# nianticlabs/panoptic-forecasting

Measured on AMD Instinct MI355X. Metric: forecast frames/sec @1024x2048, 3-in->dt=3 bg, higher is better.
Workload: dtype f32 as 2 fp16 terms/operand, 3 MFMA products, f32 accumulate (strict f32: fp32_only); 1 GPU; configs[1] bg short-term forecast 3-in dt=3 @1024x2048: 3 warp/splats + HarDNet-70 + upsample/argmax; resident_frames_per_gpu=128, streams=4, sub_batch=32, launch=hipGraph replay, sub-batches staggered, weights=random-init, calibrated (tests/golden/calib_seed1234.json), world=1, device=AMD Radeon Graphics, backend=single process

## Files before the change

include/pfhip.h:

```cpp
#ifndef PFHIP_H
#define PFHIP_H

#include <stddef.h>
#include <stdint.h>

#ifdef __cplusplus
extern "C" {
#endif

#define PF_OK 0
#define PF_EINVAL (-1)
#define PF_EWORKSPACE (-2)
#define PF_EBLOB (-3)
#define PF_EHIP (-4)
#define PF_EUNSUPPORTED (-5)

typedef struct pf_plan pf_plan;

int pf_version(void);
const char *pf_last_error(void);

#define PF_SPLAT_PER_FRAME 1
#define PF_SPLAT_PER_SAMPLE_SENTINEL 2
int pf_warp_splat_workspace(int B, int T, int H, int W, int per_frame, size_t *bytes);
// ... 128 lines not shown
int pf_train_param_count(const pf_train *t, size_t *n_floats);
int pf_train_param_layout(const pf_train *t, int op_index, size_t *w_off, size_t *aux_off, int *has_bn);
int pf_train_workspace(const pf_train *t, int B, int H, int W, int out_h, int out_w, size_t *bytes);
int pf_train_forward_backward(const pf_train *t, float *theta, float *grad, int accumulate_grads, const void *seg, int seg_is_i64,
                              const float *depth, const uint8_t *depth_mask, float depth_mean, float depth_std, int T,
                              const float *x_dense, int B, int H, int W, const void *labels, int labels_i64, int out_h, int out_w,
                              int ignore_index, float loss_scale, float bn_momentum, float bn_eps, int update_running_stats,
                              double *out3, void *ws, size_t ws_bytes, void *stream);
int pf_train_tensor_view(const pf_train *t, const char *name, int want_grad, int B, int H, int W, int out_h, int out_w,
                         size_t *ws_offset, int *channels, int *h, int *w);
int pf_sgd_workspace(size_t *bytes);
int pf_sgd_step(float *theta, float *grad, float *momentum_buf, const uint8_t *trainable, size_t n, float lr, float momentum,
                float weight_decay, float clip_norm, float clip_value, int first_step, void *ws, size_t ws_bytes, void *stream);

int pf_hardnet_tensor_view(const pf_plan *plan, const char *name, int B, int H, int W,
                           size_t *ws_offset, int *channels, int *h, int *w);
int pf_hardnet_tensor_read(const pf_plan *plan, const char *name, int B, int H, int W, const void *ws, float *dst, void *stream);
int pf_s4_pack(const float *src, void *dst, int B, int C, int H, int W, unsigned *status, void *stream);
int pf_s4_unpack(const void *src, float *dst, int B, int C, int H, int W, void *stream);
int pf_hardnet_flops(const pf_plan *plan, int H, int W, double *flops);

int pf_profile_enable(int on);
int pf_profile_collect(void);
int pf_profile_get(int i, char *label, size_t label_cap, int *launches, double *total_ms, double *flops,
                   double *bytes);

int pf_debug_force_conv(int kind, int p0, int p1, int p2);
int pf_debug_conv_decision(int ks, int stride, int cin, int cout, int hout, int wout, int B, int need, int flags, int rounds,
                           int *out, int cap);
int pf_debug_net_choice(int what, const int *iargs, int n_iargs, const float *fargs, int n_fargs, char *label, size_t label_cap,
                        long long *out, int cap);
int pf_debug_conv_ranges(int form, int ks, int kc, int pad, int n_src, int n_cases, const int *choff, const int *ch, const int *ctotal,
                         int src_begin, int src_end, int *out, size_t cap);
int pf_debug_pack_conv(int layout, int ks, int stride, int cin, int cout, int n_src, const int *choff, const int *ch, int pad_sources,
                       int rem, int tiles, int chunks, const float *w, float *out, size_t cap, size_t *n_floats);
int pf_debug_plan_arena(const void *blob, size_t bytes, int in_ch, int n_cls, float *out, size_t cap, size_t *n_floats,
                        long long *table, int table_ops);
int pf_debug_plan_tail(const void *blob, size_t bytes, int in_ch, int n_cls, float *out, size_t cap, size_t *n_floats,
                       long long *table, int table_ops);
int pf_debug_plan_down(const void *blob, size_t bytes, int in_ch, int n_cls, float *out, size_t cap, size_t *n_floats,
                       long long *table, int table_ops);
int pf_debug_plan_wide(int form, const void *blob, size_t bytes, int in_ch, int n_cls, float *out, size_t cap, size_t *n_floats,
                       long long *table, int table_ops);
int pf_debug_hardnet_schedule(const void *blob, size_t bytes, int in_ch, int n_cls, int B, int H, int W, int out_h, int out_w, int stem_T,
                              int table_batch, unsigned char *formats, int cap_formats, int *n_formats, long long *steps, int cap_steps,
                              int *n_steps);
int pf_debug_train_plan(const void *blob, size_t bytes, int in_ch, int n_cls, int B, int H, int W, int out_h, int out_w,
                        long long *regions, int cap_regions, int *n_regions, int *steps, int cap_steps, int *n_steps, int *slots_streams);
int pf_debug_fg_schedule(int N, int T_in, int T_out, int flags, long long *regions, int cap_regions, int *n_regions, long long *steps,
                         char *labels, int cap_steps, int *n_steps);
int pf_debug_label_scan_span(unsigned long long addr_a, unsigned long long addr_b, int esz_a, int esz_b, int align_a, int align_b,
                             unsigned long long n, int P, unsigned long long *out5);
int pf_debug_probe_read(long long *host64);

#ifdef __cplusplus
}
#endif
#endif
```

panoptic-forecasting_amd/csrc/warp_splat.hip:

```cpp
#include "pf_common.h"
#include "pf_prof.h"
#include <cstdlib>

#ifndef PF_PROBE
#define PF_PROBE 0
#endif
#if PF_PROBE
#define RPROBE(i) do { if (threadIdx.x == 0 && blockIdx.x == 100 && blockIdx.y == 1 && blockIdx.z == 0 && a.probe) a.probe[i] = wall_clock64(); } while (0)
#else
#define RPROBE(i) do { } while (0)
#endif

namespace pf {
long long *probe_buffer();

constexpr unsigned long long kEmpty = ~0ull;
constexpr int kThreads = 256;
constexpr int kRThreads = 512;
constexpr int kRMinWaves = 8;
constexpr int kRHalves = kRThreads / 256;
constexpr int kSrcTH = 16, kSrcTW = 64;
constexpr int kDstTH = 32, kDstTW = 128;
constexpr int kScan = 256;
constexpr int kScanBatches = 8;
constexpr int kListCap = 64;
constexpr int kFlight = 2;
constexpr int kIdFrameShift = 20;
constexpr int kZSlots = 64;

struct SplatArgs {
    const float *depth;
    const uint8_t *mask;
    const uint8_t *seg;
    const float *Kinv, *E, *Tt, *Einv, *K;
    int4 *bbox;
    unsigned *zmax_part;
    uint8_t *inv_mark;
    uint2 *proj;
    unsigned *count;
    unsigned *lists;
    uint8_t *out_seg;
    float *out_depth;
    long long *out_r2d;
    int B, T_total, t_first, T, H, W, C, per_frame;
    int zgroups_per_sample;
    int stx, sty;
    int dtx, dty;
    long long *probe;
};

__device__ __forceinline__ unsigned float_to_ordered(float f) {
    unsigned b = __float_as_uint(f);
    return (b & 0x80000000u) ? ~b : (b | 0x80000000u);
}
__device__ __forceinline__ float ordered_to_float(unsigned k) {
    return __uint_as_float((k & 0x80000000u) ? (k & 0x7FFFFFFFu) : ~k);
}

__device__ __forceinline__ float dot3(const float *m, float a, float b, float c) {
    float acc = 0.0f;
    acc = __fadd_rn(acc, __fmul_rn(m[0], a));
    acc = __fadd_rn(acc, __fmul_rn(m[1], b));
    acc = __fadd_rn(acc, __fmul_rn(m[2], c));
    return acc;
}
__device__ __forceinline__ float dot4(const float *m, float a, float b, float c, float d) {
    float acc = 0.0f;
    acc = __fadd_rn(acc, __fmul_rn(m[0], a));
    acc = __fadd_rn(acc, __fmul_rn(m[1], b));
    acc = __fadd_rn(acc, __fmul_rn(m[2], c));
    acc = __fadd_rn(acc, __fmul_rn(m[3], d));
    return acc;
}

// ... 135 lines not shown
        for (int k = 0; k < 4; ++k)
#pragma unroll
            for (int i = 0; i < 4; ++i) vv[k][i] = dot4(E + 4 * i, c[k][0], c[k][1], c[k][2], 1.0f);
    }
    {
        float Tm[16];
        fetch_rows(after(relaunder((const float *)pT), relaunder((const float *)pT), vv[3][3]), Tm);
#pragma unroll
        for (int k = 0; k < 4; ++k)
#pragma unroll
            for (int i = 0; i < 4; ++i) w[k][i] = dot4(Tm + 4 * i, vv[k][0], vv[k][1], vv[k][2], vv[k][3]);
    }
    {
        float Einv[16];
        fetch_rows(after(relaunder((const float *)pEinv), relaunder((const float *)pEinv), w[3][3]), Einv);
#pragma unroll
        for (int k = 0; k < 4; ++k)
#pragma unroll
            for (int i = 0; i < 4; ++i) e[k][i] = dot4(Einv + 4 * i, w[k][0], w[k][1], w[k][2], w[k][3]);
    }
    float K[9];
    fetch_rows(after(relaunder((const float *)pK), relaunder((const float *)pK), e[3][3]), K);
#pragma unroll
    for (int k = 0; k < 4; ++k) {
        const float px = __fdiv_rn(e[k][0], e[k][3]), py = __fdiv_rn(e[k][1], e[k][3]), z = __fdiv_rn(e[k][2], e[k][3]);
        const float q0 = dot3(K + 0, px, py, z), q1 = dot3(K + 3, px, py, z), q2 = dot3(K + 6, px, py, z);
        p[k] = finish(__fdiv_rn(q0, q2), __fdiv_rn(q1, q2), z, m[k], Wf, Hf);
    }
}

__device__ __forceinline__ void load4(const SplatArgs &a, long long base, int x, int y, float d[4], bool m[4]) {
    const long long i = base + (long long)y * a.W + x;
    if ((a.W & 3) == 0 && x + 3 < a.W) {
        const float4 dv = *reinterpret_cast<const float4 *>(a.depth + i);
        const uchar4 mv = *reinterpret_cast<const uchar4 *>(a.mask + i);
        d[0] = dv.x; d[1] = dv.y; d[2] = dv.z; d[3] = dv.w;
        m[0] = mv.x != 0; m[1] = mv.y != 0; m[2] = mv.z != 0; m[3] = mv.w != 0;
    } else {
#pragma unroll
        for (int k = 0; k < 4; ++k) {
            const bool in = x + k < a.W;
            d[k] = in ? a.depth[i + k] : 1.0f;
            m[k] = in ? a.mask[i + k] != 0 : false;
        }
    }
}

__global__ __launch_bounds__(kThreads) void bin_kernel(SplatArgs a) {
    const int tile = blockIdx.x, tl = blockIdx.y, b = blockIdx.z;
    const int t = a.t_first + tl;
    const int ty0 = (tile / a.stx) * kSrcTH, tx0 = (tile % a.stx) * kSrcTW;
    const long long N = (long long)a.H * a.W;
    const long long in_base = ((long long)b * a.T_total + t) * N;
    const int y = ty0 + (threadIdx.x >> 4), x = tx0 + (threadIdx.x & 15) * 4;
    float d[4] = {1.0f, 1.0f, 1.0f, 1.0f};
    bool m[4] = {false, false, false, false};
    if (y < a.H && x < a.W) load4(a, in_base, x, y, d, m);
    const GlobalF pKinv = (GlobalF)a.Kinv + b * 9, pK = (GlobalF)a.K + b * 9, pE = (GlobalF)a.E + b * 16, pEinv = (GlobalF)a.Einv + b * 16,
                  pT = (GlobalF)a.Tt + ((long long)b * a.T_total + t) * 16;
    const bool affine = camera_affine(pKinv, pE, pT, pEinv, pK);
    const bool skewfree = camera_skewfree(pKinv, pK);
    const int g = a.per_frame ? tl : 0, G = a.per_frame ? a.T : 1;
    uint8_t *mark = a.inv_mark + ((long long)b * G + g) * N;
    long long *r2d = a.out_r2d ? a.out_r2d + ((long long)b * a.T + tl) * N * 2 : nullptr;
    const float Wf = (float)a.W, Hf = (float)a.H;

    float zmax = -INFINITY;
    int bx0 = 0x7fffffff, by0 = 0x7fffffff, bx1 = -1, by1 = -1;
    if (y < a.H && x < a.W) {
        uint2 *pj = a.proj + ((long long)b * a.T + tl) * N + (long long)y * a.W + x;
        unsigned pk[8];
        Proj p4[4];
        const bool fast_done = affine && skewfree && project4_fast<true>(pKinv, pE, pT, pEinv, pK, x, y, d, m, Wf, Hf, p4);
        if (!fast_done) {
            project4_full(pKinv, pE, pT, pEinv, pK, x, y, d, m, Wf, Hf, p4);
        }
#pragma unroll
        for (int k = 0; k < 4; ++k) {
            if (x + k >= a.W) break;
            const Proj p = p4[k];
            zmax = fmaxf(zmax, p.z);
            pk[2 * k] = __float_as_uint(p.z);
            pk[2 * k + 1] = (unsigned)p.x0 | ((unsigned)p.y0 << 13) | ((unsigned)(p.x1 != p.x0) << 26) |
                            ((unsigned)(p.y1 != p.y0) << 27) | ((unsigned)p.valid << 28);
            if ((a.W & 3) != 0) pj[k] = make_uint2(pk[2 * k], pk[2 * k + 1]);
            if (r2d) {
                const long long n = (long long)y * a.W + x + k;
                r2d[n * 2] = p.x0;
                r2d[n * 2 + 1] = p.y0;
            }
            if (p.valid) {
                bx0 = min(bx0, p.x0); by0 = min(by0, p.y0);
                bx1 = max(bx1, p.x1); by1 = max(by1, p.y1);
            } else {
                const unsigned o00 = (unsigned)p.y0 * (unsigned)a.W + (unsigned)p.x0, dxo = (unsigned)(p.x1 - p.x0);
                const unsigned o10 = (unsigned)p.y1 * (unsigned)a.W + (unsigned)p.x0;
                if (dxo) {
                    __builtin_memcpy(mark + o00, "\1\1", 2);
                    if (o10 != o00) __builtin_memcpy(mark + o10, "\1\1", 2);
                } else {
                    mark[o00] = 1;
                    if (o10 != o00) mark[o10] = 1;
                }
            }
        }
        if ((a.W & 3) == 0) {
            reinterpret_cast<uint4 *>(pj)[0] = make_uint4(pk[0], pk[1], pk[2], pk[3]);
            reinterpret_cast<uint4 *>(pj)[1] = make_uint4(pk[4], pk[5], pk[6], pk[7]);
        }
    }
    typedef unsigned short u16x2 __attribute__((ext_vector_type(2)));
    typedef short i16x2 __attribute__((ext_vector_type(2)));
    u16x2 bmin = {(unsigned short)min(bx0, 0xFFFF), (unsigned short)min(by0, 0xFFFF)};
    i16x2 bmax = {(short)bx1, (short)by1};
#define PF_DPP_STEP(ctrl, rmask)                                                                                              \
    {                                                                                                                         \
        zmax = fmaxf(zmax, __int_as_float(__builtin_amdgcn_update_dpp(__float_as_int(zmax), __float_as_int(zmax), ctrl, rmask, 0xF, false))); \
        const int mn = __builtin_bit_cast(int, bmin), mx = __builtin_bit_cast(int, bmax);                                     \
        bmin = __builtin_elementwise_min(bmin, __builtin_bit_cast(u16x2, __builtin_amdgcn_update_dpp(mn, mn, ctrl, rmask, 0xF, false))); \
        bmax = __builtin_elementwise_max(bmax, __builtin_bit_cast(i16x2, __builtin_amdgcn_update_dpp(mx, mx, ctrl, rmask, 0xF, false))); \
    }
    PF_DPP_STEP(0xB1, 0xF)
    PF_DPP_STEP(0x4E, 0xF)
    PF_DPP_STEP(0x141, 0xF)
    PF_DPP_STEP(0x140, 0xF)
    PF_DPP_STEP(0x142, 0xA)
    PF_DPP_STEP(0x143, 0xC)
#undef PF_DPP_STEP
    __shared__ float zred[kThreads / 64];
    __shared__ int bred[kThreads / 64][2];
    if ((threadIdx.x & 63) == 63) {
        const int w = threadIdx.x >> 6;
        zred[w] = zmax;
        bred[w][0] = __builtin_bit_cast(int, bmin);
        bred[w][1] = __builtin_bit_cast(int, bmax);
    }
    __syncthreads();
    zmax = zred[0];
    bmin = __builtin_bit_cast(u16x2, bred[0][0]);
    bmax = __builtin_bit_cast(i16x2, bred[0][1]);
#pragma unroll
    for (int w = 1; w < kThreads / 64; ++w) {
        zmax = fmaxf(zmax, zred[w]);
        bmin = __builtin_elementwise_min(bmin, __builtin_bit_cast(u16x2, bred[w][0]));
        bmax = __builtin_elementwise_max(bmax, __builtin_bit_cast(i16x2, bred[w][1]));
    }
    bx0 = bmin[0] == 0xFFFF ? 0x7fffffff : (int)bmin[0];
    by0 = bmin[1] == 0xFFFF ? 0x7fffffff : (int)bmin[1];
    bx1 = bmax[0];
    by1 = bmax[1];
    if (threadIdx.x == 0) {
        const long long ntile = (long long)a.stx * a.sty;
        atomicMax(&a.zmax_part[(b * a.zgroups_per_sample + (a.per_frame ? tl : 0)) * kZSlots + ((tile + b) & (kZSlots - 1))], float_to_ordered(zmax));
        a.bbox[((long long)b * a.T + tl) * ntile + tile] = make_int4(bx0, by0, bx1, by1);
    }
    if (bx1 >= 0) {
        const int ndst = a.dtx * a.dty;
        const long long dbase = ((long long)b * G + g) * ndst;
        const unsigned id = ((unsigned)(a.per_frame ? 0 : tl) << kIdFrameShift) | (unsigned)tile;
        const int dtx0 = bx0 / kDstTW, dty0 = by0 / kDstTH;
        const int ntx = bx1 / kDstTW - dtx0 + 1, nt = ntx * (by1 / kDstTH - dty0 + 1);
        for (int j = threadIdx.x; j < nt; j += kThreads) {
            const long long dst = dbase + (dty0 + j / ntx) * a.dtx + dtx0 + j % ntx;
            const unsigned slot = atomicAdd(&a.count[dst], 1u);
            if (slot < (unsigned)kListCap) a.lists[dst * kListCap + slot] = id;
        }
    }
}

__global__ __launch_bounds__(kRThreads, kRMinWaves) void raster_kernel(SplatArgs a) {
    __shared__ unsigned long long zb[kDstTH * kDstTW];
    __shared__ unsigned short list[kScan * kScanBatches];
    __shared__ unsigned ent[kListCap];
    __shared__ int list_n;
    __shared__ float sentinel_s;

    const int dtile = blockIdx.x, g = blockIdx.y, b = blockIdx.z;
    const int G = a.per_frame ? a.T : 1, Tg = a.per_frame ? 1 : a.T;
    const int dy0 = (dtile / a.dtx) * kDstTH, dx0 = (dtile % a.dtx) * kDstTW;
    const int dy1 = min(dy0 + kDstTH, a.H) - 1, dx1 = min(dx0 + kDstTW, a.W) - 1;
    const long long N = (long long)a.H * a.W;
    const long long P = (long long)Tg * N;
    const int ntile = a.stx * a.sty;

    RPROBE(0);
    [[maybe_unused]] int n_hits_total = 0;
    for (int i = threadIdx.x; i < kDstTH * kDstTW; i += kRThreads) zb[i] = kEmpty;
    const int lt = threadIdx.x & 255, half = threadIdx.x >> 8;

    if (threadIdx.x < 64) {
        unsigned m = a.zmax_part[(b * a.zgroups_per_sample + (a.per_frame ? g : 0)) * kZSlots + threadIdx.x];
#pragma unroll
        for (int o = 32; o > 0; o >>= 1) m = max(m, (unsigned)__shfl_xor((int)m, o));
        if (threadIdx.x == 0) sentinel_s = __fadd_rn(ordered_to_float(m), 1.0f);
    }

    auto splat4 = [&](const unsigned (&pk)[8], int x, int y, unsigned ebase) {
        const unsigned e_first = ebase + (unsigned)y * (unsigned)a.W + (unsigned)x;
        const unsigned Pu1 = (unsigned)P;
#pragma unroll
        for (int k = 0; k < 4; ++k) {
            const unsigned f = pk[2 * k + 1];
            if (!((f >> 28) & 1u)) continue;
            const unsigned rx0 = (f & 8191u) - (unsigned)dx0, ry0 = ((f >> 13) & 8191u) - (unsigned)dy0;
            const unsigned fx = (f >> 26) & 1u, fy = (f >> 27) & 1u;
            const unsigned rx1 = rx0 + fx, ry1 = ry0 + fy;
            const bool in_x0 = rx0 < (unsigned)kDstTW, in_x1 = rx1 < (unsigned)kDstTW && fx != 0u;
            const bool in_y0 = ry0 < (unsigned)kDstTH, in_y1 = ry1 < (unsigned)kDstTH && fy != 0u;
            const unsigned e0 = e_first + (unsigned)k;
            const unsigned long long khi = (unsigned long long)pk[2 * k] << 32;
            if (in_x0 && in_y0) atomicMin(&zb[ry0 * kDstTW + rx0], khi | e0);
            if (in_x0 && in_y1) atomicMin(&zb[ry1 * kDstTW + rx0], khi | (e0 + Pu1));
            if (in_x1 && in_y0) atomicMin(&zb[ry0 * kDstTW + rx1], khi | (e0 + 2u * Pu1));
            if (in_x1 && in_y1) atomicMin(&zb[ry1 * kDstTW + rx1], khi | (e0 + 3u * Pu1));
        }
    };
    auto load4 = [&](const uint2 *pbase, int stx, int sty, unsigned (&pk)[8], int &x, int &y) {
        y = sty * kSrcTH + (lt >> 4);
        x = stx * kSrcTW + (lt & 15) * 4;
#pragma unroll
        for (int k = 0; k < 8; ++k) pk[k] = 0u;
        if (stx < 0 || y >= a.H || x >= a.W) return;
        const uint2 *pj = pbase + (long long)y * a.W + x;
        if ((a.W & 3) == 0) {
            const uint4 q0 = reinterpret_cast<const uint4 *>(pj)[0], q1 = reinterpret_cast<const uint4 *>(pj)[1];
            pk[0] = q0.x; pk[1] = q0.y; pk[2] = q0.z; pk[3] = q0.w;
            pk[4] = q1.x; pk[5] = q1.y; pk[6] = q1.z; pk[7] = q1.w;
        } else {
#pragma unroll
            for (int k = 0; k < 4; ++k) {
                const uint2 q = x + k < a.W ? pj[k] : make_uint2(0u, 0u);
                pk[2 * k] = q.x; pk[2 * k + 1] = q.y;
            }
        }
    };
    const int ndst = a.dtx * a.dty;
    const long long dslot = ((long long)b * G + g) * ndst + dtile;
    const unsigned cnt = a.count[dslot];
    if (cnt <= (unsigned)kListCap) {
        if (threadIdx.x < cnt) {
            const unsigned e = a.lists[dslot * kListCap + threadIdx.x], st = e & ((1u << kIdFrameShift) - 1u), row = st / (unsigned)a.stx;
            ent[threadIdx.x] = (e & ~((1u << kIdFrameShift) - 1u)) | (row << 10) | (st - row * (unsigned)a.stx);
        }
        __syncthreads();
        for (int li = 0; li < (int)cnt; li += kFlight * kRHalves) {
            unsigned pk[kFlight][8];
            int xs[kFlight], ys[kFlight];
            unsigned eb[kFlight];
#pragma unroll
            for (int j = 0; j < kFlight; ++j) {
                const int le = li + j * kRHalves + half;
                const unsigned e = le < (int)cnt ? ent[le] : 0u;
                const int tt = (int)(e >> kIdFrameShift), sx = le < (int)cnt ? (int)(e & 1023u) : -1, sy = (int)((e >> 10) & 1023u);
                const int tl = a.per_frame ? g : tt;
                eb[j] = (unsigned)tt * (unsigned)N;
                load4(a.proj + ((long long)b * a.T + tl) * N, sx, sy, pk[j], xs[j], ys[j]);
            }
#pragma unroll
            for (int j = 0; j < kFlight; ++j) splat4(pk[j], xs[j], ys[j], eb[j]);
        }
    } else {
    for (int tt = 0; tt < Tg; ++tt) {
        const int tl = a.per_frame ? g : tt;
        const int4 *boxes = a.bbox + ((long long)b * a.T + tl) * ntile;
        const uint2 *pbase = a.proj + ((long long)b * a.T + tl) * N;
        const unsigned ebase = (unsigned)tt * (unsigned)N;
        for (int s0 = 0; s0 < ntile; s0 += kScan * kScanBatches) {
            __syncthreads();
            if (threadIdx.x == 0) list_n = 0;
            __syncthreads();
#pragma unroll
            for (int j = 0; j < kScanBatches; ++j) {
                const int s = s0 + j * kScan + lt;
                if (s < ntile && half == 0) {
                    const int4 bb = boxes[s];
                    if (bb.x <= dx1 && bb.z >= dx0 && bb.y <= dy1 && bb.w >= dy0) list[atomicAdd(&list_n, 1)] = (unsigned short)(s - s0);
                }
            }
            __syncthreads();
            const int n_hit = list_n;
            n_hits_total += n_hit;
            RPROBE(4);
            for (int li = 0; li < n_hit; li += 4 * kRHalves) {
                unsigned pk[4][8];
                int xs[4], ys[4];
#pragma unroll
                for (int j = 0; j < 4; ++j) {
                    const int le = li + j * kRHalves + half;
                    const int st = le < n_hit ? s0 + list[le] : -1;
                    load4(pbase, st < 0 ? -1 : st % a.stx, st < 0 ? 0 : st / a.stx, pk[j], xs[j], ys[j]);
                }
#pragma unroll
                for (int j = 0; j < 4; ++j) splat4(pk[j], xs[j], ys[j], ebase);
            }
        }
    }
    }
    __syncthreads();
    RPROBE(1);
#if PF_PROBE
    if (threadIdx.x == 0 && blockIdx.x == 100 && blockIdx.y == 1 && blockIdx.z == 0 && a.probe) a.probe[3] = n_hits_total;
#endif

    const float sentinel = sentinel_s;
    const uint8_t *mark = a.inv_mark + ((long long)b * G + g) * N;
    const long long out_base = ((long long)b * G + g) * N;
    const long long seg_base = ((long long)b * a.T_total + a.t_first + (a.per_frame ? g : 0)) * N;
    const int C = a.C;
    const unsigned Pu = (unsigned)P;
    const uint8_t *segp = a.seg + seg_base * C;
    float *outd = a.out_depth + out_base;
    uint8_t *outs = a.out_seg + out_base * C;
#pragma unroll
    for (int it = 0; it < kDstTH * kDstTW / 4 / kRThreads; ++it) {
        const int i4 = it * kRThreads + threadIdx.x;
        const int y = dy0 + i4 / (kDstTW / 4), x = dx0 + (i4 % (kDstTW / 4)) * 4;
        if (y >= a.H || x >= a.W) continue;
        const unsigned n0 = (unsigned)y * (unsigned)a.W + (unsigned)x;
        unsigned zbits[4], src[4];
        bool empty[4];
        uint8_t mk[4], sg[4];
#pragma unroll
        for (int k = 0; k < 4; ++k) {
            const unsigned long long key = zb[i4 * 4 + k];
            zbits[k] = (unsigned)(key >> 32);
            empty[k] = zbits[k] == 0xFFFFFFFFu;
            unsigned e = (unsigned)key;
            e -= e >= 2u * Pu ? 2u * Pu : 0u;
            e -= e >= Pu ? Pu : 0u;
            src[k] = empty[k] ? 0u : e;
        }
        if ((a.W & 3) == 0) {
            const uchar4 mv = *reinterpret_cast<const uchar4 *>(mark + n0);
            mk[0] = mv.x; mk[1] = mv.y; mk[2] = mv.z; mk[3] = mv.w;
        } else {
#pragma unroll
            for (int k = 0; k < 4; ++k) mk[k] = x + k < a.W ? mark[n0 + k] : (uint8_t)0;
        }
#pragma unroll
        for (int k = 0; k < 4; ++k) sg[k] = C == 1 ? segp[src[k]] : (uint8_t)0;
        float dep[4];
#pragma unroll
        for (int k = 0; k < 4; ++k) {
            dep[k] = !empty[k] ? __uint_as_float(zbits[k]) : (mk[k] ? sentinel : -1.0f);
            if (empty[k]) sg[k] = 0;
        }
        if ((a.W & 3) == 0) {
            *reinterpret_cast<float4 *>(outd + n0) = make_float4(dep[0], dep[1], dep[2], dep[3]);
            if (C == 1) *reinterpret_cast<uchar4 *>(outs + n0) = make_uchar4(sg[0], sg[1], sg[2], sg[3]);
        } else {
#pragma unroll
            for (int k = 0; k < 4; ++k)
                if (x + k < a.W) {
                    outd[n0 + k] = dep[k];
                    if (C == 1) outs[n0 + k] = sg[k];
                }
        }
        if (C != 1) {
#pragma unroll
            for (int k = 0; k < 4; ++k)
                if (x + k < a.W)
                    for (int c = 0; c < C; ++c)
                        outs[(size_t)(n0 + k) * C + c] = !empty[k] ? segp[(size_t)src[k] * C + c] : (uint8_t)0;
        }
    }
    RPROBE(2);
}

struct SplatLayout {
    size_t bbox_off, zmax_off, count_off, mark_off, mark_bytes, proj_off, lists_off, total;
    int stx, sty, dtx, dty;
};

static SplatLayout splat_layout(int B, int T, int H, int W, int per_frame) {
    SplatLayout L;
    L.stx = (W + kSrcTW - 1) / kSrcTW; L.sty = (H + kSrcTH - 1) / kSrcTH;
    L.dtx = (W + kDstTW - 1) / kDstTW; L.dty = (H + kDstTH - 1) / kDstTH;
    const size_t ntile = (size_t)L.stx * L.sty, N = (size_t)H * W;
    L.bbox_off = 0;
    L.zmax_off = align_up(L.bbox_off + (size_t)B * T * ntile * sizeof(int4), 256);
    const size_t ndst = (size_t)L.dtx * L.dty, G = per_frame ? T : 1;
    L.count_off = align_up(L.zmax_off + (size_t)B * T * kZSlots * sizeof(unsigned), 256);
    L.mark_off = align_up(L.count_off + B * G * ndst * sizeof(unsigned), 256);
    L.mark_bytes = (size_t)B * G * N;
    L.proj_off = align_up(L.mark_off + L.mark_bytes, 256);
    L.lists_off = align_up(L.proj_off + (size_t)B * T * N * sizeof(uint2), 256);
    L.total = align_up(L.lists_off + B * G * ndst * kListCap * sizeof(unsigned), 256);
    return L;
}

}

extern "C" int pf_warp_splat_workspace(int B, int T, int H, int W, int per_frame, size_t *bytes) {
    if (!bytes || B <= 0 || T <= 0 || H <= 0 || W <= 0)
        return pf::fail(PF_EINVAL, "pf_warp_splat_workspace: bad dims B=%d T=%d H=%d W=%d", B, T, H, W);
    if (4ll * T * H * W >= (1ll << 32))
        return pf::fail(PF_EUNSUPPORTED, "pf_warp_splat: 4*T*H*W must be < 2^32 (element index packs in 32 bits)");
    if (H > 8192 || W > 8192 || T >= 4096)
        return pf::fail(PF_EUNSUPPORTED, "pf_warp_splat: H and W must be <= 8192 (13-bit bin coordinates) and T < 4096");
    *bytes = pf::splat_layout(B, T, H, W, per_frame & PF_SPLAT_PER_FRAME).total;
    return PF_OK;
}

extern "C" int pf_warp_splat(const float *depth, const uint8_t *depth_mask, const uint8_t *seg,
                             int seg_channels, const float *Kinv, const float *E, const float *T_tgt,
                             const float *Einv, const float *K, int B, int T_total, int t_first, int T,
                             int H, int W, int per_frame, uint8_t *out_seg, float *out_depth,
                             int64_t *out_result2d, void *ws, size_t ws_bytes, void *stream) {
    if (!depth || !depth_mask || !seg || !Kinv || !E || !T_tgt || !Einv || !K || !out_seg || !out_depth || !ws)
        return pf::fail(PF_EINVAL, "pf_warp_splat: null pointer argument");
    if (seg_channels != 1 && seg_channels != 3)
        return pf::fail(PF_EINVAL, "pf_warp_splat: seg_channels must be 1 or 3, got %d", seg_channels);
    if (B <= 0 || T <= 0 || H <= 0 || W <= 0 || t_first < 0 || t_first + T > T_total)
        return pf::fail(PF_EINVAL, "pf_warp_splat: bad dims B=%d T_total=%d t_first=%d T=%d H=%d W=%d", B,
                        T_total, t_first, T, H, W);
    size_t need = 0;
    int rc = pf_warp_splat_workspace(B, T, H, W, per_frame, &need);
    if (rc) return rc;
    if (ws_bytes < need)
        return pf::fail(PF_EWORKSPACE, "pf_warp_splat: workspace %zu B < required %zu B", ws_bytes, need);

    const pf::SplatLayout L = pf::splat_layout(B, T, H, W, per_frame & PF_SPLAT_PER_FRAME);
    pf::SplatArgs a;
    a.depth = depth; a.mask = depth_mask; a.seg = seg;
    a.Kinv = Kinv; a.E = E; a.Tt = T_tgt; a.Einv = Einv; a.K = K;
    a.bbox = (int4 *)((char *)ws + L.bbox_off);
    a.zmax_part = (unsigned *)((char *)ws + L.zmax_off);
    a.inv_mark = (uint8_t *)ws + L.mark_off;
    a.proj = (uint2 *)((char *)ws + L.proj_off);
    a.count = (unsigned *)((char *)ws + L.count_off);
    a.lists = (unsigned *)((char *)ws + L.lists_off);
    a.out_seg = out_seg; a.out_depth = out_depth; a.out_r2d = (long long *)out_result2d;
    a.B = B; a.T_total = T_total; a.t_first = t_first; a.T = T; a.H = H; a.W = W; a.C = seg_channels;
    a.per_frame = (per_frame & PF_SPLAT_PER_FRAME) ? 1 : 0;
    a.zgroups_per_sample = (per_frame & PF_SPLAT_PER_SAMPLE_SENTINEL) ? (a.per_frame ? T : 1) : 0;
    a.stx = L.stx; a.sty = L.sty; a.dtx = L.dtx; a.dty = L.dty;
    a.probe = nullptr;
#if PF_PROBE
    static const bool splat_probe = pf::ab_env("PF_PROBE") != nullptr;
    a.probe = splat_probe ? pf::probe_buffer() : nullptr;
#endif
    hipStream_t s = (hipStream_t)stream;
    const int G = a.per_frame ? T : 1;

    const double src_px = (double)B * T * H * W, dst_px = (double)B * G * H * W;
    {
        pf::ProfScope ps(s, "inv_mark_memset", 0, (double)L.mark_bytes);
        if (int rc = pf::launch_zero_fill(a.zmax_part, (L.mark_off - L.zmax_off) + L.mark_bytes, s)) return rc;
    }
    {
        pf::ProfScope ps(s, "pf::bin_kernel(pf::SplatArgs)", 0, src_px * (5.0 + (out_result2d ? 16.0 : 0.0)));
        hipLaunchKernelGGL(pf::bin_kernel, dim3(L.stx * L.sty, T, B), dim3(pf::kThreads), 0, s, a);
        PF_LAUNCH_CHECK("bin_kernel");
    }
    {
        pf::ProfScope ps(s, "pf::raster_kernel(pf::SplatArgs)", 0, dst_px * (2.0 * seg_channels + 4.0));
        hipLaunchKernelGGL(pf::raster_kernel, dim3(L.dtx * L.dty, G, B), dim3(pf::kRThreads), 0, s, a);
        PF_LAUNCH_CHECK("raster_kernel");
    }
    return PF_OK;
}
```

panoptic-forecasting_amd/lib.py:

```python
import ctypes
import os

_HERE = os.path.dirname(os.path.abspath(__file__))
LIB_PATH = os.environ.get('PF_LIBPFHIP') or os.path.join(_HERE, 'csrc', 'libpfhip.so')

_c = ctypes
_vp, _i, _f, _sz = _c.c_void_p, _c.c_int, _c.c_float, _c.c_size_t

SIGNATURES = {
    'pf_version': (_i, []),
    'pf_last_error': (_c.c_char_p, []),
    'pf_warp_splat_workspace': (_i, [_i, _i, _i, _i, _i, _c.POINTER(_sz)]),
    'pf_warp_splat': (_i, [_vp, _vp, _vp, _i, _vp, _vp, _vp, _vp, _vp, _i, _i, _i, _i, _i, _i, _i,
                           _vp, _vp, _vp, _vp, _sz, _vp]),
    'pf_hardnet_plan_create': (_i, [_vp, _sz, _i, _i, _c.POINTER(_vp)]),
    'pf_hardnet_plan_destroy': (None, [_vp]),
    'pf_hardnet_workspace': (_i, [_vp, _i, _i, _i, _c.POINTER(_sz)]),
    'pf_bg_forward': (_i, [_vp, _vp, _i, _vp, _vp, _f, _f, _i, _f, _f, _i, _i, _i, _i, _i, _i,
                           _vp, _i, _vp, _vp, _vp, _sz, _vp]),
    'pf_hardnet_forward_dense': (_i, [_vp, _vp, _i, _i, _i, _i, _i, _vp, _i, _vp, _vp, _vp, _sz, _vp]),
    'pf_hardnet_tensor_view': (_i, [_vp, _c.c_char_p, _i, _i, _i, _c.POINTER(_sz), _c.POINTER(_i),
                                    _c.POINTER(_i), _c.POINTER(_i)]),
    'pf_hardnet_tensor_read': (_i, [_vp, _c.c_char_p, _i, _i, _i, _vp, _vp, _vp]),
    'pf_hardnet_status': (_i, [_vp, _c.POINTER(_c.c_uint), _vp]),
# ... 15 lines not shown
    'pf_panoptic_max_ids': (_i, []),
    'pf_pq_workspace': (_i, [_i, _c.POINTER(_sz)]),
    'pf_pq_table_slots': (_i, []),
    'pf_pq_accumulate': (_i, [_vp, _i, _vp, _i, _i, _i, _i, _i, _i, _i, _vp, _vp, _vp, _sz, _vp]),
    'pf_pq_status': (_i, [_vp, _vp, _c.POINTER(_i)]),
    'pf_pq_status_reset': (_i, [_vp, _vp]),
    'pf_confusion_workspace': (_i, [_i, _c.POINTER(_sz)]),
    'pf_confusion_chunk_pixels': (_i, []),
    'pf_confusion_accumulate': (_i, [_vp, _i, _vp, _i, _i, _i, _i, _i, _i, _vp, _vp, _vp, _sz, _vp]),
    'pf_confusion_status': (_i, [_vp, _vp, _c.POINTER(_i)]),
    'pf_confusion_status_reset': (_i, [_vp, _vp]),
    'pf_iiou_workspace': (_i, [_i, _c.POINTER(_sz)]),
    'pf_iiou_chunk_pixels': (_i, []),
    'pf_iiou_accumulate': (_i, [_vp, _i, _vp, _i, _i, _i, _i, _i, _i, _vp, _vp, _vp, _vp, _vp, _sz, _vp]),
    'pf_iiou_status': (_i, [_vp, _vp, _c.POINTER(_i)]),
    'pf_iiou_status_reset': (_i, [_vp, _vp]),
    'pf_bg_dense_input': (_i, [_vp, _i, _i, _vp, _vp, _f, _f, _i, _i, _i, _i, _vp, _vp]),
    'pf_seg_loss_workspace': (_i, [_i, _i, _i, _c.POINTER(_sz)]),
    'pf_seg_loss': (_i, [_vp, _i, _i, _i, _i, _vp, _i, _i, _i, _i, _vp, _vp, _sz, _vp]),
    'pf_train_create': (_i, [_vp, _sz, _i, _i, _c.POINTER(_vp)]),
    'pf_train_destroy': (None, [_vp]),
    'pf_train_autotune': (_i, [_vp, _i]),
    'pf_train_tuned_shapes': (_i, [_vp, _c.POINTER(_i), _i, _c.POINTER(_i)]),
    'pf_train_path_stats': (_i, [_vp, _c.POINTER(_i), _i, _c.POINTER(_i)]),
    'pf_train_param_count': (_i, [_vp, _c.POINTER(_sz)]),
    'pf_train_param_layout': (_i, [_vp, _i, _c.POINTER(_sz), _c.POINTER(_sz), _c.POINTER(_i)]),
    'pf_train_workspace': (_i, [_vp, _i, _i, _i, _i, _i, _c.POINTER(_sz)]),
    'pf_train_forward_backward': (_i, [_vp, _vp, _vp, _i, _vp, _i, _vp, _vp, _f, _f, _i, _vp, _i, _i, _i, _vp, _i, _i, _i, _i, _f, _f,
                                       _f, _i, _vp, _vp, _sz, _vp]),
    'pf_train_tensor_view': (_i, [_vp, _c.c_char_p, _i, _i, _i, _i, _i, _i, _c.POINTER(_sz), _c.POINTER(_i), _c.POINTER(_i),
                                  _c.POINTER(_i)]),
    'pf_sgd_workspace': (_i, [_c.POINTER(_sz)]),
    'pf_sgd_step': (_i, [_vp, _vp, _vp, _vp, _sz, _f, _f, _f, _f, _f, _i, _vp, _sz, _vp]),
    'pf_fg_weights_size': (_i, [_i, _c.POINTER(_sz), _c.POINTER(_sz)]),
    'pf_fg_pack': (_i, [_vp, _vp, _i, _vp]),
    'pf_fg_workspace': (_i, [_i, _i, _i, _i, _c.POINTER(_sz)]),
    'pf_fg_forward': (_i, [_vp, _i, _i, _i, _i, _i, _vp, _vp, _vp, _vp, _vp, _vp, _vp, _vp, _vp, _vp, _vp, _vp, _vp, _vp,
                           _vp, _sz, _vp]),
    'pf_fg_pair_workspace': (_i, [_i, _i, _i, _c.POINTER(_sz)]),
    'pf_fg_status': (_i, [_vp, _c.POINTER(_c.c_uint), _vp]),
    'pf_fg_status_reset': (_i, [_vp, _vp]),
    'pf_odom_weights_size': (_i, [_i, _c.POINTER(_sz), _c.POINTER(_sz)]),
    'pf_odom_pack': (_i, [_vp, _vp, _i, _vp]),
    'pf_odom_forward': (_i, [_vp, _i, _i, _i, _i, _vp, _vp, _vp, _vp]),
    'pf_odom_train_workspace': (_i, [_i, _i, _i, _i, _c.POINTER(_sz)]),
    'pf_odom_train_forward': (_i, [_vp, _i, _i, _i, _i, _vp, _vp, _vp, _vp, _sz, _vp]),
    'pf_odom_backward': (_i, [_vp, _i, _i, _i, _i, _vp, _vp, _vp, _vp, _vp, _sz, _vp, _vp]),
    'pf_set_option': (_i, [_c.c_char_p, _i]),
    'pf_hardnet_plan_set_option': (_i, [_vp, _c.c_char_p, _i]),
    'pf_debug_force_conv': (_i, [_i, _i, _i, _i]),
    'pf_debug_conv_decision': (_i, [_i, _i, _i, _i, _i, _i, _i, _i, _i, _i, _c.POINTER(_i), _i]),
    'pf_debug_net_choice': (_i, [_i, _c.POINTER(_i), _i, _c.POINTER(_f), _i, _c.c_char_p, _sz, _c.POINTER(_c.c_longlong), _i]),
    'pf_debug_probe_read': (_i, [_c.POINTER(_c.c_longlong)]),
    'pf_debug_conv_ranges': (_i, [_i, _i, _i, _i, _i, _i, _vp, _vp, _vp, _i, _i, _vp, _sz]),
    'pf_debug_pack_conv': (_i, [_i, _i, _i, _i, _i, _i, _vp, _vp, _i, _i, _i, _i, _vp, _vp, _sz, _c.POINTER(_sz)]),
    'pf_debug_plan_arena': (_i, [_vp, _sz, _i, _i, _vp, _sz, _c.POINTER(_sz), _vp, _i]),
    'pf_debug_plan_tail': (_i, [_vp, _sz, _i, _i, _vp, _sz, _c.POINTER(_sz), _vp, _i]),
    'pf_debug_plan_down': (_i, [_vp, _sz, _i, _i, _vp, _sz, _c.POINTER(_sz), _vp, _i]),
    'pf_debug_plan_wide': (_i, [_i, _vp, _sz, _i, _i, _vp, _sz, _c.POINTER(_sz), _vp, _i]),
    'pf_debug_train_plan':(_i, [_vp, _sz, _i, _i, _i, _i, _i, _i, _i, _vp, _i, _c.POINTER(_i), _vp, _i, _c.POINTER(_i), _vp]),
    'pf_debug_hardnet_schedule': (_i, [_vp, _sz, _i, _i, _i, _i, _i, _i, _i, _i, _i, _vp, _i, _c.POINTER(_i), _vp, _i, _c.POINTER(_i)]),
    'pf_debug_fg_schedule': (_i, [_i, _i, _i, _i, _vp, _i, _c.POINTER(_i), _vp, _vp, _i, _c.POINTER(_i)]),
    'pf_debug_label_scan_span': (_i, [_c.c_ulonglong, _c.c_ulonglong, _i, _i, _i, _i, _c.c_ulonglong, _i, _c.POINTER(_c.c_ulonglong)]),
    'pf_profile_enable': (_i, [_i]),
    'pf_profile_collect': (_i, []),
    'pf_profile_get': (_i, [_i, _c.c_char_p, _sz, _c.POINTER(_i), _c.POINTER(_c.c_double),
                            _c.POINTER(_c.c_double), _c.POINTER(_c.c_double)]),
}


def profile(enable):
    check(load().pf_profile_enable(int(enable)), 'pf_profile_enable')


def profile_results():
    L = load()
    n = L.pf_profile_collect()
    if n < 0:
        check(n, 'pf_profile_collect')
    out = []
    for i in range(n):
        buf = ctypes.create_string_buffer(160)
        la, ms, fl, by = _i(), _c.c_double(), _c.c_double(), _c.c_double()
        check(L.pf_profile_get(i, buf, 160, ctypes.byref(la), ctypes.byref(ms), ctypes.byref(fl), ctypes.byref(by)),
              'pf_profile_get')
        out.append({'label': buf.value.decode(), 'launches': la.value, 'ms': ms.value, 'flops': fl.value,
                    'bytes': by.value})
    return out

_lib = None


class PfError(RuntimeError):
    pass


def load():
    global _lib
    if _lib is None:
        import torch
        if not os.path.exists(LIB_PATH):
            raise PfError('%s not found: build it with `python -c "import __graft_entry__ as g; g.build()"` '
                          '(make -C panoptic-forecasting_amd/csrc). There is no fallback path.' % LIB_PATH)
        lib = ctypes.CDLL(LIB_PATH)
        for name, (res, args) in SIGNATURES.items():
            fn = getattr(lib, name)
# ... 22 lines not shown
```

panoptic-forecasting_amd/pc_transform_model.py:

```python
import ctypes

import torch

from . import lib as _lib
from .model_api import BaseModel


PF_SPLAT_PER_FRAME, PF_SPLAT_PER_SAMPLE_SENTINEL = 1, 2


def host_inverse(m):
    return torch.inverse(m.detach().float().cpu()).contiguous().to(m.device)


def add_camera_inverses(inputs):
    K, E = inputs.get('intrinsics'), inputs.get('extrinsics')
    if not (torch.is_tensor(K) and torch.is_tensor(E)) or K.is_cuda or E.is_cuda:
        return inputs
    out = dict(inputs)
    if out.get('intrinsics_inv') is None:
        out['intrinsics_inv'] = torch.inverse(K.detach().float()).contiguous()
    if out.get('extrinsics_inv') is None:
        out['extrinsics_inv'] = torch.inverse(E.detach().float()).contiguous()
    return out
# ... 18 lines not shown
        if m.is_cuda:
            check = self.verify and not capturing
            if hit is not None and not check and not capturing and self.verify_every > 0:
                n = self._hits.get(key, 0)
                self._hits[key] = n + 1
                check = n % self.verify_every == 0
        else:
            check = True
        if hit is not None and check and not torch.equal(m, hit[2]):
            hit = None
        if hit is None:
            self._d.pop(key, None)
            self._hits.pop(key, None)
            if len(self._d) >= self.capacity:
                old = next(iter(self._d))
                self._d.pop(old)
                self._hits.pop(old, None)
            self._dev_misses += int(m.is_cuda)
            if self._dev_misses == 9 and not self._warned:
                import warnings
                self._warned = True
                warnings.warn('panoptic_forecasting_amd: camera matrices arrive as new device tensors: every predict() reads them '
                              'back and inverts on the host (two stream synchronisations).  Take the inverses on the host batch '
                              'with pc_transform_model.add_camera_inverses(inputs) before moving it to the GPU (INTEGRATION.md A).')
            hit = (m, host_inverse(m), m.detach().clone())
            self._d[key] = hit
        return hit[1]


_inverse_cache = InverseCache()


def _as_u8(mask):
    if mask.dtype == torch.bool:
        return mask.contiguous().view(torch.uint8)
    return mask if mask.dtype == torch.uint8 else (mask != 0).view(torch.uint8)


def _seg_as_u8(seg):
    if seg.dtype == torch.uint8:
        return seg
    if seg.is_floating_point():
        raise _lib.PfError('seg must be an integer label map or a u8 image (got %s)' % seg.dtype)
    if seg.numel() and (int(seg.max()) > 255 or int(seg.min()) < 0):
        raise _lib.PfError('seg holds values outside 0..255 (min %d, max %d): the device splat gathers u8 payloads'
                           % (int(seg.min()), int(seg.max())))
    return seg.to(torch.uint8)


class WarpSplat:

    def __init__(self):
        self._ws = None

    def _workspace(self, b, t, h, w, per_frame, device):
        L = _lib.load()
        need = ctypes.c_size_t()
        _lib.check(L.pf_warp_splat_workspace(b, t, h, w, int(per_frame), ctypes.byref(need)),
                   'pf_warp_splat_workspace')
        if self._ws is None or self._ws.numel() < need.value or self._ws.device != device:
            self._ws = torch.empty(need.value, dtype=torch.uint8, device=device)
        return self._ws

    def __call__(self, depth, depth_mask, seg, K, E, target_T, Kinv=None, Einv=None, t_first=0, T=None,
                 per_frame=False, is_img=False, want_result2d=True, per_sample_sentinel=False):
        L = _lib.load()
        b, t_total, h, w = depth.shape
        T = t_total - t_first if T is None else T
        dev = depth.device
        depth = _lib.require_cuda(depth.float(), 'depth')
        mask = _lib.require_cuda(_as_u8(depth_mask), 'depth_mask')
        seg_dtype = seg.dtype
        seg8 = _lib.require_cuda(_seg_as_u8(seg), 'seg')
        Kinv = _inverse_cache(K) if Kinv is None else Kinv
        Einv = _inverse_cache(E) if Einv is None else Einv
        mats = [_lib.require_cuda(m.float().contiguous(), n) for m, n in
                ((Kinv, 'Kinv'), (E, 'extrinsics'), (target_T, 'target_T'), (Einv, 'Einv'), (K, 'intrinsics'))]
        c = 3 if is_img else 1
        g = T if per_frame else 1
        shape = (b, g, h, w) if per_frame else (b, h, w)
        out_seg = torch.empty(shape + ((3,) if is_img else ()), dtype=torch.uint8, device=dev)
        out_depth = torch.empty(shape, dtype=torch.float32, device=dev)
        r2d = torch.empty((b, T, h, w, 2), dtype=torch.int64, device=dev) if want_result2d else None
        ws = self._workspace(b, T, h, w, per_frame, dev)
        flags = (PF_SPLAT_PER_FRAME if per_frame else 0) | (PF_SPLAT_PER_SAMPLE_SENTINEL if per_sample_sentinel else 0)
        rc = L.pf_warp_splat(depth.data_ptr(), mask.data_ptr(), seg8.data_ptr(), c,
                             mats[0].data_ptr(), mats[1].data_ptr(), mats[2].data_ptr(), mats[3].data_ptr(),
                             mats[4].data_ptr(), b, t_total, t_first, T, h, w, flags,
                             out_seg.data_ptr(), out_depth.data_ptr(),
                             r2d.data_ptr() if r2d is not None else None,
                             ws.data_ptr(), ws.numel(), _lib.stream_ptr())
        _lib.check(rc, 'pf_warp_splat')
        if seg_dtype != torch.uint8:
            out_seg = out_seg.to(seg_dtype)
        return out_seg, out_depth, r2d


class PCTransformModel(BaseModel):
    def __init__(self, params):
        super().__init__()
        self.ind = params['model'].get('only_this_ind')
        self.is_img = params['model'].get('is_img')
        self.debug = params['model'].get('debug')
        self.per_sample_sentinel = bool(params['model'].get('per_sample_sentinel', False))
        self._splat = WarpSplat()

    @torch.no_grad()
    def predict(self, inputs, labels=None):
        depth = inputs['depth']
        t_first, T = (0, depth.shape[1]) if self.ind is None else (self.ind, 1)
        seg, dep, r2d = self._splat(depth, inputs['depth_mask'], inputs['seg'], inputs['intrinsics'],
                                    inputs['extrinsics'], inputs['target_T'],
                                    Kinv=inputs.get('intrinsics_inv'), Einv=inputs.get('extrinsics_inv'),
                                    t_first=t_first, T=T, per_frame=False, is_img=bool(self.is_img),
                                    per_sample_sentinel=self.per_sample_sentinel)
        return {'seg': seg, 'result2d': r2d, 'depth': dep}
```

Measured before the change: 2951 frames/s.

## Bin splat sources per wave-sized 8x32 block instead of whole 16x64 tile

The bin kernel now computes a bounding box per wave (an 8x32 sub-block) instead of reducing to one box per 16x64 tile. Each sub-block is appended only to the destination bins its own tighter box overlaps, and the resolve kernel walks lists at wave granularity, one entry per wave instead of per half-block. The aim is fewer false-positive source loads and splats in each destination tile. In exchange the bbox array is four times larger, there are more list entries and atomics, and per-bin lists may hit the 64-entry cap more often, which sends those bins to the slower fallback scan. A debug API for reading per-bin counts is also added.

```diff
diff --git a/include/pfhip.h b/include/pfhip.h
--- a/include/pfhip.h
+++ b/include/pfhip.h
@@ -204,6 +204,8 @@
 int pf_debug_label_scan_span(unsigned long long addr_a, unsigned long long addr_b, int esz_a, int esz_b, int align_a, int align_b,
                              unsigned long long n, int P, unsigned long long *out5);
 int pf_debug_probe_read(long long *host64);
+int pf_debug_splat_counts(const void *ws, size_t ws_bytes, int B, int T, int H, int W, int per_frame, unsigned *host_counts, size_t cap,
+                          size_t *n_counts, void *stream);
 
 #ifdef __cplusplus
 }
diff --git a/panoptic-forecasting_amd/csrc/warp_splat.hip b/panoptic-forecasting_amd/csrc/warp_splat.hip
--- a/panoptic-forecasting_amd/csrc/warp_splat.hip
+++ b/panoptic-forecasting_amd/csrc/warp_splat.hip
@@ -18,8 +18,11 @@
 constexpr int kThreads = 256;
 constexpr int kRThreads = 512;
 constexpr int kRMinWaves = 8;
-constexpr int kRHalves = kRThreads / 256;
+constexpr int kRWaves = kRThreads / 64;
 constexpr int kSrcTH = 16, kSrcTW = 64;
+constexpr int kBlkH = 8, kBlkW = 32;
+constexpr int kTileBlocks = (kSrcTH / kBlkH) * (kSrcTW / kBlkW);
+static_assert(kTileBlocks == kThreads / 64 && kSrcTW / kBlkW == 2, "one wave per block, two blocks per tile row");
 constexpr int kDstTH = 32, kDstTW = 128;
 constexpr int kScan = 256;
 constexpr int kScanBatches = 8;
@@ -261,7 +264,8 @@
     const int ty0 = (tile / a.stx) * kSrcTH, tx0 = (tile % a.stx) * kSrcTW;
     const long long N = (long long)a.H * a.W;
     const long long in_base = ((long long)b * a.T_total + t) * N;
-    const int y = ty0 + (threadIdx.x >> 4), x = tx0 + (threadIdx.x & 15) * 4;
+    const int wave = threadIdx.x >> 6, lane = threadIdx.x & 63;
+    const int y = ty0 + (wave >> 1) * kBlkH + (lane >> 3), x = tx0 + (wave & 1) * kBlkW + (lane & 7) * 4;
     float d[4] = {1.0f, 1.0f, 1.0f, 1.0f};
     bool m[4] = {false, false, false, false};
     if (y < a.H && x < a.W) load4(a, in_base, x, y, d, m);
@@ -338,42 +342,40 @@
 #undef PF_DPP_STEP
     __shared__ float zred[kThreads / 64];
     __shared__ int bred[kThreads / 64][2];
-    if ((threadIdx.x & 63) == 63) {
-        const int w = threadIdx.x >> 6;
-        zred[w] = zmax;
-        bred[w][0] = __builtin_bit_cast(int, bmin);
-        bred[w][1] = __builtin_bit_cast(int, bmax);
+    if (lane == 63) {
+        const long long ntile = (long long)a.stx * a.sty;
+        zred[wave] = zmax;
+        bred[wave][0] = __builtin_bit_cast(int, bmin);
+        bred[wave][1] = __builtin_bit_cast(int, bmax);
+        a.bbox[(((long long)b * a.T + tl) * ntile + tile) * kTileBlocks + wave] =
+            make_int4(bmin[0] == 0xFFFF ? 0x7fffffff : (int)bmin[0], bmin[1] == 0xFFFF ? 0x7fffffff : (int)bmin[1], bmax[0], bmax[1]);
     }
     __syncthreads();
-    zmax = zred[0];
-    bmin = __builtin_bit_cast(u16x2, bred[0][0]);
-    bmax = __builtin_bit_cast(i16x2, bred[0][1]);
-#pragma unroll
-    for (int w = 1; w < kThreads / 64; ++w) {
-        zmax = fmaxf(zmax, zred[w]);
-        bmin = __builtin_elementwise_min(bmin, __builtin_bit_cast(u16x2, bred[w][0]));
-        bmax = __builtin_elementwise_max(bmax, __builtin_bit_cast(i16x2, bred[w][1]));
-    }
-    bx0 = bmin[0] == 0xFFFF ? 0x7fffffff : (int)bmin[0];
-    by0 = bmin[1] == 0xFFFF ? 0x7fffffff : (int)bmin[1];
-    bx1 = bmax[0];
-    by1 = bmax[1];
-    if (threadIdx.x == 0) {
-        const long long ntile = (long long)a.stx * a.sty;
+    if (wave != 0) return;
+    if (lane == 0) {
+        zmax = zred[0];
+#pragma unroll
+        for (int w = 1; w < kThreads / 64; ++w) zmax = fmaxf(zmax, zred[w]);
         atomicMax(&a.zmax_part[(b * a.zgroups_per_sample + (a.per_frame ? tl : 0)) * kZSlots + ((tile + b) & (kZSlots - 1))], float_to_ordered(zmax));
-        a.bbox[((long long)b * a.T + tl) * ntile + tile] = make_int4(bx0, by0, bx1, by1);
-    }
-    if (bx1 >= 0) {
+    }
+    {
+        const int blk = lane >> 4, jx = lane & 3, jy = (lane >> 2) & 3;
+        bmin = __builtin_bit_cast(u16x2, bred[blk][0]);
+        bmax = __builtin_bit_cast(i16x2, bred[blk][1]);
+        bx0 = bmin[0]; by0 = bmin[1];
+        bx1 = bmax[0]; by1 = bmax[1];
+        if (bx1 < 0) return;
         const int ndst = a.dtx * a.dty;
         const long long dbase = ((long long)b * G + g) * ndst;
-        const unsigned id = ((unsigned)(a.per_frame ? 0 : tl) << kIdFrameShift) | (unsigned)tile;
+        const unsigned id = ((unsigned)(a.per_frame ? 0 : tl) << kIdFrameShift) | (unsigned)(tile * kTileBlocks + blk);
         const int dtx0 = bx0 / kDstTW, dty0 = by0 / kDstTH;
-        const int ntx = bx1 / kDstTW - dtx0 + 1, nt = ntx * (by1 / kDstTH - dty0 + 1);
-        for (int j = threadIdx.x; j < nt; j += kThreads) {
-            const long long dst = dbase + (dty0 + j / ntx) * a.dtx + dtx0 + j % ntx;
-            const unsigned slot = atomicAdd(&a.count[dst], 1u);
-            if (slot < (unsigned)kListCap) a.lists[dst * kListCap + slot] = id;
-        }
+        const int ntx = bx1 / kDstTW - dtx0 + 1, nty = by1 / kDstTH - dty0 + 1;
+        for (int oy = jy; oy < nty; oy += 4)
+            for (int ox = jx; ox < ntx; ox += 4) {
+                const long long dst = dbase + (dty0 + oy) * a.dtx + dtx0 + ox;
+                const unsigned slot = atomicAdd(&a.count[dst], 1u);
+                if (slot < (unsigned)kListCap) a.lists[dst * kListCap + slot] = id;
+            }
     }
 }
 
@@ -390,12 +392,12 @@
     const int dy1 = min(dy0 + kDstTH, a.H) - 1, dx1 = min(dx0 + kDstTW, a.W) - 1;
     const long long N = (long long)a.H * a.W;
     const long long P = (long long)Tg * N;
-    const int ntile = a.stx * a.sty;
+    const int nblock = a.stx * a.sty * kTileBlocks;
 
     RPROBE(0);
     [[maybe_unused]] int n_hits_total = 0;
     for (int i = threadIdx.x; i < kDstTH * kDstTW; i += kRThreads) zb[i] = kEmpty;
-    const int lt = threadIdx.x & 255, half = threadIdx.x >> 8;
+    const int lane = threadIdx.x & 63, wave = threadIdx.x >> 6;
 
     if (threadIdx.x < 64) {
         unsigned m = a.zmax_part[(b * a.zgroups_per_sample + (a.per_frame ? g : 0)) * kZSlots + threadIdx.x];
@@ -424,12 +426,12 @@
             if (in_x1 && in_y1) atomicMin(&zb[ry1 * kDstTW + rx1], khi | (e0 + 3u * Pu1));
         }
     };
-    auto load4 = [&](const uint2 *pbase, int stx, int sty, unsigned (&pk)[8], int &x, int &y) {
-        y = sty * kSrcTH + (lt >> 4);
-        x = stx * kSrcTW + (lt & 15) * 4;
+    auto load4 = [&](const uint2 *pbase, int bcol, int brow, unsigned (&pk)[8], int &x, int &y) {
+        y = brow * kBlkH + (lane >> 3);
+        x = bcol * kBlkW + (lane & 7) * 4;
 #pragma unroll
         for (int k = 0; k < 8; ++k) pk[k] = 0u;
-        if (stx < 0 || y >= a.H || x >= a.W) return;
+        if (bcol < 0 || y >= a.H || x >= a.W) return;
         const uint2 *pj = pbase + (long long)y * a.W + x;
         if ((a.W & 3) == 0) {
             const uint4 q0 = reinterpret_cast<const uint4 *>(pj)[0], q1 = reinterpret_cast<const uint4 *>(pj)[1];
@@ -448,17 +450,18 @@
     const unsigned cnt = a.count[dslot];
     if (cnt <= (unsigned)kListCap) {
         if (threadIdx.x < cnt) {
-            const unsigned e = a.lists[dslot * kListCap + threadIdx.x], st = e & ((1u << kIdFrameShift) - 1u), row = st / (unsigned)a.stx;
-            ent[threadIdx.x] = (e & ~((1u << kIdFrameShift) - 1u)) | (row << 10) | (st - row * (unsigned)a.stx);
+            const unsigned e = a.lists[dslot * kListCap + threadIdx.x], sb = e & ((1u << kIdFrameShift) - 1u);
+            const unsigned st = sb / kTileBlocks, w = sb % kTileBlocks, row = st / (unsigned)a.stx;
+            ent[threadIdx.x] = (e & ~((1u << kIdFrameShift) - 1u)) | ((row * 2u + (w >> 1)) << 10) | ((st - row * (unsigned)a.stx) * 2u + (w & 1u));
         }
         __syncthreads();
-        for (int li = 0; li < (int)cnt; li += kFlight * kRHalves) {
+        for (int li = 0; li < (int)cnt; li += kFlight * kRWaves) {
             unsigned pk[kFlight][8];
             int xs[kFlight], ys[kFlight];
             unsigned eb[kFlight];
 #pragma unroll
             for (int j = 0; j < kFlight; ++j) {
-                const int le = li + j * kRHalves + half;
+                const int le = li + j * kRWaves + wave;
                 const unsigned e = le < (int)cnt ? ent[le] : 0u;
                 const int tt = (int)(e >> kIdFrameShift), sx = le < (int)cnt ? (int)(e & 1023u) : -1, sy = (int)((e >> 10) & 1023u);
                 const int tl = a.per_frame ? g : tt;
@@ -471,17 +474,17 @@
     } else {
     for (int tt = 0; tt < Tg; ++tt) {
         const int tl = a.per_frame ? g : tt;
-        const int4 *boxes = a.bbox + ((long long)b * a.T + tl) * ntile;
+        const int4 *boxes = a.bbox + ((long long)b * a.T + tl) * nblock;
         const uint2 *pbase = a.proj + ((long long)b * a.T + tl) * N;
         const unsigned ebase = (unsigned)tt * (unsigned)N;
-        for (int s0 = 0; s0 < ntile; s0 += kScan * kScanBatches) {
+        for (int s0 = 0; s0 < nblock; s0 += kScan * kScanBatches) {
             __syncthreads();
             if (threadIdx.x == 0) list_n = 0;
             __syncthreads();
 #pragma unroll
             for (int j = 0; j < kScanBatches; ++j) {
-                const int s = s0 + j * kScan + lt;
-                if (s < ntile && half == 0) {
+                const int s = s0 + j * kScan + (int)threadIdx.x;
+                if (s < nblock && threadIdx.x < kScan) {
                     const int4 bb = boxes[s];
                     if (bb.x <= dx1 && bb.z >= dx0 && bb.y <= dy1 && bb.w >= dy0) list[atomicAdd(&list_n, 1)] = (unsigned short)(s - s0);
                 }
@@ -490,14 +493,14 @@
             const int n_hit = list_n;
             n_hits_total += n_hit;
             RPROBE(4);
-            for (int li = 0; li < n_hit; li += 4 * kRHalves) {
+            for (int li = 0; li < n_hit; li += 4 * kRWaves) {
                 unsigned pk[4][8];
                 int xs[4], ys[4];
 #pragma unroll
                 for (int j = 0; j < 4; ++j) {
-                    const int le = li + j * kRHalves + half;
-                    const int st = le < n_hit ? s0 + list[le] : -1;
-                    load4(pbase, st < 0 ? -1 : st % a.stx, st < 0 ? 0 : st / a.stx, pk[j], xs[j], ys[j]);
+                    const int le = li + j * kRWaves + wave;
+                    const int sb = le < n_hit ? s0 + list[le] : -1, st = sb / kTileBlocks, w = sb % kTileBlocks;
+                    load4(pbase, sb < 0 ? -1 : (st % a.stx) * 2 + (w & 1), sb < 0 ? 0 : (st / a.stx) * 2 + (w >> 1), pk[j], xs[j], ys[j]);
                 }
 #pragma unroll
                 for (int j = 0; j < 4; ++j) splat4(pk[j], xs[j], ys[j], ebase);
@@ -587,7 +590,7 @@
     L.dtx = (W + kDstTW - 1) / kDstTW; L.dty = (H + kDstTH - 1) / kDstTH;
     const size_t ntile = (size_t)L.stx * L.sty, N = (size_t)H * W;
     L.bbox_off = 0;
-    L.zmax_off = align_up(L.bbox_off + (size_t)B * T * ntile * sizeof(int4), 256);
+    L.zmax_off = align_up(L.bbox_off + (size_t)B * T * ntile * kTileBlocks * sizeof(int4), 256);
     const size_t ndst = (size_t)L.dtx * L.dty, G = per_frame ? T : 1;
     L.count_off = align_up(L.zmax_off + (size_t)B * T * kZSlots * sizeof(unsigned), 256);
     L.mark_off = align_up(L.count_off + B * G * ndst * sizeof(unsigned), 256);
@@ -607,6 +610,10 @@
         return pf::fail(PF_EUNSUPPORTED, "pf_warp_splat: 4*T*H*W must be < 2^32 (element index packs in 32 bits)");
     if (H > 8192 || W > 8192 || T >= 4096)
         return pf::fail(PF_EUNSUPPORTED, "pf_warp_splat: H and W must be <= 8192 (13-bit bin coordinates) and T < 4096");
+    const long long brows = (H + pf::kBlkH - 1) / pf::kBlkH, bcols = (W + pf::kBlkW - 1) / pf::kBlkW;
+    const long long tiles = ((H + pf::kSrcTH - 1) / pf::kSrcTH) * (long long)((W + pf::kSrcTW - 1) / pf::kSrcTW);
+    if (tiles * pf::kTileBlocks > (1ll << pf::kIdFrameShift) || brows > 1024 || bcols > 1024)
+        return pf::fail(PF_EUNSUPPORTED, "pf_warp_splat: %lld source blocks (%lld x %lld) do not fit the list entry", tiles * pf::kTileBlocks, brows, bcols);
     *bytes = pf::splat_layout(B, T, H, W, per_frame & PF_SPLAT_PER_FRAME).total;
     return PF_OK;
 }
@@ -669,3 +676,22 @@
     }
     return PF_OK;
 }
+
+extern "C" int pf_debug_splat_counts(const void *ws, size_t ws_bytes, int B, int T, int H, int W, int per_frame, unsigned *host_counts,
+                                     size_t cap, size_t *n_counts, void *stream) {
+    if (!ws || !n_counts) return pf::fail(PF_EINVAL, "pf_debug_splat_counts: null pointer argument");
+    size_t need = 0;
+    if (int rc = pf_warp_splat_workspace(B, T, H, W, per_frame, &need)) return rc;
+    if (ws_bytes < need)
+        return pf::fail(PF_EWORKSPACE, "pf_debug_splat_counts: workspace %zu B < required %zu B", ws_bytes, need);
+    const pf::SplatLayout L = pf::splat_layout(B, T, H, W, per_frame & PF_SPLAT_PER_FRAME);
+    const size_t n = (size_t)B * ((per_frame & PF_SPLAT_PER_FRAME) ? T : 1) * L.dtx * L.dty;
+    *n_counts = n;
+    if (!host_counts) return PF_OK;
+    if (cap < n) return pf::fail(PF_EINVAL, "pf_debug_splat_counts: room for %zu counts, %zu needed", cap, n);
+    hipStream_t s = (hipStream_t)stream;
+    if (hipMemcpyAsync(host_counts, (const char *)ws + L.count_off, n * sizeof(unsigned), hipMemcpyDeviceToHost, s) != hipSuccess ||
+        hipStreamSynchronize(s) != hipSuccess)
+        return pf::fail(PF_EHIP, "pf_debug_splat_counts: copying the counts failed");
+    return PF_OK;
+}
diff --git a/panoptic-forecasting_amd/lib.py b/panoptic-forecasting_amd/lib.py
--- a/panoptic-forecasting_amd/lib.py
+++ b/panoptic-forecasting_amd/lib.py
@@ -91,6 +91,7 @@
     'pf_debug_conv_decision': (_i, [_i, _i, _i, _i, _i, _i, _i, _i, _i, _i, _c.POINTER(_i), _i]),
     'pf_debug_net_choice': (_i, [_i, _c.POINTER(_i), _i, _c.POINTER(_f), _i, _c.c_char_p, _sz, _c.POINTER(_c.c_longlong), _i]),
     'pf_debug_probe_read': (_i, [_c.POINTER(_c.c_longlong)]),
+    'pf_debug_splat_counts': (_i, [_vp, _sz, _i, _i, _i, _i, _i, _vp, _sz, _c.POINTER(_sz), _vp]),
     'pf_debug_conv_ranges': (_i, [_i, _i, _i, _i, _i, _i, _vp, _vp, _vp, _i, _i, _vp, _sz]),
     'pf_debug_pack_conv': (_i, [_i, _i, _i, _i, _i, _i, _vp, _vp, _i, _i, _i, _i, _vp, _vp, _sz, _c.POINTER(_sz)]),
     'pf_debug_plan_arena': (_i, [_vp, _sz, _i, _i, _vp, _sz, _c.POINTER(_sz), _vp, _i]),
diff --git a/panoptic-forecasting_amd/pc_transform_model.py b/panoptic-forecasting_amd/pc_transform_model.py
--- a/panoptic-forecasting_amd/pc_transform_model.py
+++ b/panoptic-forecasting_amd/pc_transform_model.py
@@ -94,6 +94,7 @@
 
     def __init__(self):
         self._ws = None
+        self._last = None
 
     def _workspace(self, b, t, h, w, per_frame, device):
         L = _lib.load()
@@ -133,9 +134,21 @@
                              r2d.data_ptr() if r2d is not None else None,
                              ws.data_ptr(), ws.numel(), _lib.stream_ptr())
         _lib.check(rc, 'pf_warp_splat')
+        self._last = (b, T, h, w, flags)
         if seg_dtype != torch.uint8:
             out_seg = out_seg.to(seg_dtype)
         return out_seg, out_depth, r2d
+
+    def list_counts(self):
+        L = _lib.load()
+        b, T, h, w, flags = self._last
+        n = ctypes.c_size_t()
+        args = (self._ws.data_ptr(), self._ws.numel(), b, T, h, w, flags)
+        _lib.check(L.pf_debug_splat_counts(*args, None, 0, ctypes.byref(n), _lib.stream_ptr()), 'pf_debug_splat_counts')
+        host = (ctypes.c_uint * n.value)()
+        _lib.check(L.pf_debug_splat_counts(*args, host, n.value, ctypes.byref(n), _lib.stream_ptr()), 'pf_debug_splat_counts')
+        g = T if flags & PF_SPLAT_PER_FRAME else 1
+        return torch.tensor(list(host), dtype=torch.int64).view(b, g, (h + 31) // 32, (w + 127) // 128)
 
 
 class PCTransformModel(BaseModel):
```

After: 2995 frames/s, median of 6. 1.01x the previous value.
